# wells-wood-research/timed-design

Measured on AMD Instinct MI355X. Metric: residue_frames_per_sec, higher is better.
Workload: dtype f32

## Files before the change

### include/timed_hip.h

```cpp
#ifndef TIMED_HIP_H
#define TIMED_HIP_H

#include <stddef.h>
#include <stdint.h>

#ifdef __cplusplus
extern "C" {
#endif

#define TH_OK 0
#define TH_EINVAL (-1)
#define TH_EIO (-2)
#define TH_EHIP (-3)
#define TH_EUNSUP (-4)
#define TH_ENOMEM (-5)
#define TH_ECOMM (-6)
#define TH_EBUSY (-7)

#define TH_F32 0
#define TH_F64 1
#define TH_U8 2
#define TH_BOOL 3
#define TH_F16 4

#define TH_LOAD_DEFAULT 0u
#define TH_LOAD_NO_FUSE 1u
#define TH_LOAD_NO_MFMA 2u
#define TH_LOAD_KEEP_ALL 4u

#define TH_PREDICT_DEFAULT 0u
#define TH_PREDICT_LOGITS 1u
#define TH_PREDICT_OUT_DEVICE 2u
#define TH_PREDICT_IN_DEVICE 4u

typedef struct th_model th_model;
typedef struct th_comm th_comm;

int th_version(void);
const char* th_last_error(void);
int th_device_count(int* n_out);
int th_host_cpus(void);
int th_device_info(int device, char* name, size_t name_len, char* arch, size_t arch_len, int* cus);

int th_model_load(const char* pack_path, int device, unsigned flags, th_model** out);
int th_model_load_mem(const void* pack, size_t nbytes, int device, unsigned flags, th_model** out);
void th_model_free(th_model* m);
int th_model_info(const th_model* m, int dims[4], int* n_classes);
int th_model_cost(const th_model* m, double* algo_flops, double* exec_flops, int* n_steps);
int th_model_set_chunk(th_model* m, int frames_per_chunk);
int th_conv_gl_row_tiles(int64_t rows);

int th_predict(th_model* m, const void* frames, int dtype, int64_t n, float* probs_out, unsigned flags);
int th_predict_async(th_model* m, const void* frames, int dtype, int64_t n, float* probs_out, unsigned flags, int* ticket);
int th_predict_wait(th_model* m, int ticket);
#define TH_SPARSE_MAGIC "THSPF001"
int th_predict_sparse_async(th_model* m, const void* blob, size_t blob_bytes, float* probs_out, unsigned flags, int* ticket);
int th_host_alloc(size_t bytes, void** out);
int th_host_free(void* p);
int th_host_register(void* p, size_t bytes);
int th_host_unregister(void* p);
int th_predict_device(th_model* m, const void* d_frames, int dtype, int64_t n, float* d_probs, unsigned flags);
int th_model_fetch(th_model* m, const char* layer_name, int64_t n, float* out, int64_t out_floats);

int th_model_profile(th_model* m, int enable);
int th_model_step_info(const th_model* m, int i, char* label, size_t label_len, double* ms, int64_t* launches,
                       double* flops_per_frame, double* exec_flops_per_frame, double* bytes_per_frame);
int th_model_step_direct_flops(const th_model* m, int i, double* direct_flops_per_frame);

int th_model_guard_info(const th_model* m, int* state, double* max_dlogit, double* logit_scale, char* note, size_t note_len);

int th_model_knobs(const th_model* m, char* buf, size_t buf_len);

int th_dev_alloc(int device, size_t bytes, void** d_out);
int th_dev_free(int device, void* d);
int th_dev_upload(int device, void* d_dst, const void* h_src, size_t bytes);
int th_dev_download(int device, void* h_dst, const void* d_src, size_t bytes);
int th_dev_sync(int device);
int th_dev_synth_frames(int device, float* d_frames, int64_t n, int side, int channels, int atoms, uint64_t seed);

int th_apply_temp(const double* probs, int64_t n_res, int n_cls, double t, double* out);
int th_apply_temp_on(int device, const double* probs, int64_t n_res, int n_cls, double t, double* out);
#define TH_RNG_HOST 0
#define TH_RNG_PHILOX 1
// ... 134 lines not shown
```

### timed-design_amd/csrc/common.h

```cpp
#pragma once
#include <hip/hip_runtime.h>
#include <stdint.h>
#include <string>
#include <vector>

#include "../../include/timed_hip.h"

enum : int {
    OP_INPUT = 0, OP_CONV3D, OP_DENSE, OP_BN, OP_ACT, OP_MAXPOOL, OP_AVGPOOL, OP_GAP, OP_GMP,
    OP_FLATTEN, OP_CONCAT, OP_ADD, OP_IDENTITY
};
enum : int { ACT_LINEAR = 0, ACT_RELU, ACT_ELU, ACT_SOFTMAX, ACT_SIGMOID, ACT_TANH, ACT_LEAKY };

void th_set_error(const char* fmt, ...);
#define TH_FAIL(code, ...)          \
    do {                            \
        th_set_error(__VA_ARGS__);  \
        return (code);              \
    } while (0)
#define HIP_TRY(expr)                                                                            \
    do {                                                                                         \
        hipError_t _e = (expr);                                                                  \
        if (_e != hipSuccess) {                                                                  \
            th_set_error("%s failed: %s (%s:%d)", #expr, hipGetErrorString(_e), __FILE__, __LINE__); \
// ... 2 lines not shown
    } while (0)

#ifndef TH_KNOCKOUTS
#define TH_KNOCKOUTS 0
#endif
#if TH_KNOCKOUTS
#define TH_KNOCK_FIELD int dbg;
#define TH_KNOCK(a) ((a).dbg)
#define TH_KNOCK_SET(a, v) ((a).dbg = (v))
#else
#define TH_KNOCK_FIELD
#define TH_KNOCK(a) 0
#define TH_KNOCK_SET(a, v) ((void)0)
#endif

struct ThKnobs {
    int winograd = 1;
    int wino_split = 1;
    int wfused = 1;
    int wf_split = 1;
    int lanes = 1, lane_lag = 1;
    int guard = 1;
    int first_wino = 1;
    int first_split = 1;
    int conv_gl = 1;
    int dense_gemm = 1;
    int first_int = 1;
    int no_pool_first = 0;
    int no_tail_fuse = 0;
    int conv_notail = 0, n16_resident = 0;
    int wf_resident = 0, wf_noblk = 0;
    long long wino_piece = 0;
    int wino_b3var = 2, wino_nomid = 0;
#if TH_KNOCKOUTS
    int wf_dbg = 0, first_dbg = 0, wino_dbg = 0, conv_dbg = 0, pw_dbg = 0;
#endif
    std::string nondefault;
};
int th_knobs_read(ThKnobs* k);
inline const ThKnobs& th_knobs_of(const ThKnobs* k) { static const ThKnobs dflt; return k ? *k : dflt; }

hipError_t th_malloc_retry_impl(void** p, size_t bytes);
template <class T> inline hipError_t th_malloc_retry(T** p, size_t bytes) { return th_malloc_retry_impl(reinterpret_cast<void**>(p), bytes); }

int th_usable_cpus();

struct TView {
    float* p = nullptr;
    int D = 1, H = 1, W = 1, C = 0;
    int cs = 0;
    int coff = 0;
    int64_t fs = 0;
    int blk = 0;
    int V() const { return D * H * W; }
};

#define TH_MAX_POST 4
enum : int { POP_ACT = 1, POP_AFFINE = 2 };
struct PostOps {
    int n = 0;
    int type[TH_MAX_POST] = {0, 0, 0, 0};
    int act[TH_MAX_POST] = {0, 0, 0, 0};
    float alpha[TH_MAX_POST] = {0, 0, 0, 0};
    const float* scale[TH_MAX_POST] = {nullptr, nullptr, nullptr, nullptr};
    const float* shift[TH_MAX_POST] = {nullptr, nullptr, nullptr, nullptr};
    int monotone = 0;
// ... 62 lines not shown
int launch_conv_mfma(hipStream_t s, int64_t n, const ConvMfmaPlan& p, TView in, TView out, ConvGeom g, int Cin,
                     int Cout, const float* wpk, const float* bias, PreOp pre, PostOps post);

struct ConvN16Plan {
    int variant = -1, xc = 0;
    int pool = 0;
    int FB = 1, ZB = 0, nzb = 1;
    int Zp = 0, Hp = 0, Wp = 0;
    int Dc = 0, Hc = 0, Wc = 0;
    int rows_pf = 0, nchunks = 0;
    int geo = 0;
    int ncu = 0;
    size_t lds_bytes = 0, wpk_floats = 0;
    double exec_flops = 0;
    const ThKnobs* knobs = nullptr;
    std::string label;
};
bool conv_n16_plan(const TView& in, const TView& out_conv, const ConvGeom& g, int Cin, int Cout, int pool, const ThKnobs& kn, ConvN16Plan* plan);
void conv_n16_pack_weights(const ConvN16Plan& p, int Cin, int Cout, const float* w_keras, float* dst);
int launch_conv_n16(hipStream_t s, int64_t n, const ConvN16Plan& p, TView in, TView out, ConvGeom g, int Cin, int Cout, const float* wpk,
                    const float* bias, PreOp pre, PostOps post);

struct ConvWinoPlan {
    int P = 9;
    int Cin = 0, Cout = 0, Coutp = 0, ncb = 0;
    int Cinp = 0;
    size_t wpk_floats = 0;
    int64_t v_fpf = 0, m_fpf = 0;
    double gemm_flops = 0;
    double exec_flops = 0;
    int split = 0;
    int narrow = 0;
    int b3var = 0;
    const ThKnobs* knobs = nullptr;
    std::string label;
};
bool conv_wino_plan(const TView& in, const TView& out_conv, const ConvGeom& g, int Cin, int Cout, int scheme, int split, const ThKnobs& kn,
                    ConvWinoPlan* plan);
void conv_wino_pack_weights(const ConvWinoPlan& p, const float* w_keras, float* dst);
int launch_wino_in(hipStream_t s, int64_t n, const ConvWinoPlan& p, TView in, float* V, PreOp pre);
int launch_wino_gemm(hipStream_t s, int64_t n, const ConvWinoPlan& p, const float* V, float* M, const float* wpk);
int launch_wino_out(hipStream_t s, int64_t n, const ConvWinoPlan& p, const float* M, TView out, const float* bias, PostOps post, bool gap = false);
int launch_wino_mid(hipStream_t s, int64_t n, const ConvWinoPlan& p, const float* M, float* V_next, const float* bias, PostOps post);

struct ConvWfPlan {
    int geo = -1;
    int pool = 0;
    int Cin = 0, Cout = 0, ncb = 0, nchunks = 0;
    size_t wpk_floats = 0, lds_bytes = 0;
    double own_flops = 0;
    double exec_flops = 0;
    int ncu = 0;
    const ThKnobs* knobs = nullptr;
    std::string label;
};
bool conv_wf_plan(const TView& in, const TView& out_conv, const ConvGeom& g, int Cin, int Cout, int pool, const ThKnobs& kn, ConvWfPlan* plan);
bool conv_wf_view_ok(const TView& in);
int conv_wf_pre_kind(const PreOp& pre);
std::string conv_wf_label(const ConvWfPlan& p, const PreOp& pre);
void conv_wf_pack_weights(const ConvWfPlan& p, const float* w_keras, float* dst);
int launch_conv_wf(hipStream_t s, int64_t n, const ConvWfPlan& p, TView in, TView out, const float* wpk, const float* bias, PreOp pre,
                   PostOps post);

struct ConvWfsPlan {
    int geo = -1, pool = 0;
    int Cin = 0, Cout = 0, nkh = 0, ncp = 0;
    size_t wpk_floats = 0, lds_bytes = 0;
    double own_flops = 0, exec_flops = 0;
    int ncu = 0;
// ... 68 lines not shown
```

### timed-design_amd/csrc/conv_wino.hip

```cpp
#include "bf16x3.h"
#include "common.h"
#include "device_math.h"
#include "wino_tables.h"

#include <algorithm>
#include <cstdlib>
#include <cstring>
#include <thread>
#include <vector>

namespace {

constexpr int kZ = WINO_N;
constexpr int kNF = 64;
constexpr int kKC = 32;
constexpr int kCB = 128;

template <int R, int C>
__device__ __forceinline__ void wino_apply(const float (&T)[R][C], const float (&in)[C], float (&out)[R]) {
#pragma unroll
    for (int r = 0; r < R; ++r) {
        float acc = 0.f;
        bool first = true;
#pragma unroll
// ... 213 lines not shown
                th_act_vec<kZ * kZ>(y, a.post.act[i], a.post.alpha[i]);
            }
        }
        float u[kP][kZ];
#pragma unroll
        for (int k = 0; k < kZ; ++k) {
            float col[kZ], o[kP];
#pragma unroll
            for (int j = 0; j < kZ; ++j) col[j] = y[j * kZ + k];
            WinoTab<kP>::fwd(col, o);
#pragma unroll
            for (int aa = 0; aa < kP; ++aa) u[aa][k] = o[aa];
        }
        float* __restrict__ opos = a.V + (int64_t)z * kPos * opstride;
#pragma unroll
        for (int aa = 0; aa < kP; ++aa) {
            float o[kP];
            WinoTab<kP>::fwd(u[aa], o);
#pragma unroll
            for (int b = 0; b < kP; ++b) (opos + (int64_t)(aa * kP + b) * opstride)[ooff] = o[b];
        }
    }
}

struct WinoGemmArgs {
    const float* V; const float* U; float* M;
    int64_t Ns;
    int Cin, Coutp;
    int Cout;
    int nfb, ncb;
    int npos;
    unsigned total;
    unsigned per_xcd;
    TH_KNOCK_FIELD
};

__device__ __forceinline__ constexpr bool wino_tap_ok(int zi, int dz) { return zi - dz + 1 >= 0 && zi - dz + 1 < kZ; }

struct WinoTile {
    unsigned p, fb, cb;
    int lane, wave;
    bool active;
};

__device__ __forceinline__ bool wino_tile_index(const WinoGemmArgs& a, unsigned& L) {
    const unsigned xcd = blockIdx.x & 7u, slot = blockIdx.x >> 3;
    L = xcd * a.per_xcd + slot;
    return slot < a.per_xcd && L < a.total;
}
__device__ __forceinline__ WinoTile wino_tile(const WinoGemmArgs& a, unsigned L) {
    WinoTile t;
    t.cb = L % (unsigned)a.ncb;
    t.fb = (L / (unsigned)a.ncb) % (unsigned)a.nfb;
    t.p = L / (unsigned)(a.ncb * a.nfb);
    t.lane = threadIdx.x & 63;
    t.wave = __builtin_amdgcn_readfirstlane(threadIdx.x >> 6);
    t.active = (int)(t.cb * kCB) + t.wave * 32 < a.Cout;
    return t;
}

__global__ void __launch_bounds__(256, 2) k_wino_gemm(const WinoGemmArgs a) {
    __shared__ __attribute__((aligned(16))) float lds[kZ * kNF * kKC];
    unsigned L;
    if (!wino_tile_index(a, L)) return;
    const WinoTile t = wino_tile(a, L);
    const unsigned p = t.p, fb = t.fb, cb = t.cb;
    const int lane = t.lane, wave = t.wave;
    const int j = lane & 31, h = lane >> 5;
    const int nchunks = a.Cin / kKC;
    const int S = a.Cin / 8;
    const float4* wq = reinterpret_cast<const float4*>(a.U) + ((size_t)((p * a.ncb + cb) * 4 + wave) * S * 3) * 64 + lane;
    const float* vbase = a.V + ((int64_t)p * a.Ns + (int64_t)fb * kNF) * a.Cin;
    const int64_t zstride = (int64_t)a.npos * a.Ns * a.Cin;

    f32x16 acc[kZ][2];
#pragma unroll
    for (int z = 0; z < kZ; ++z)
#pragma unroll
        for (int rt = 0; rt < 2; ++rt)
#pragma unroll
            for (int r = 0; r < 16; ++r) acc[z][rt][r] = 0.f;
// ... 85 lines not shown
            for (int r = 0; r < 16; ++r) T[((r & 3) + 8 * (r >> 2) + 4 * h) * 36 + j] = acc[z][rt][r];
#pragma unroll
            for (int k = 0; k < 4; ++k) {
                const int row = rr + 8 * k;
                *reinterpret_cast<float4*>(mb + z * mz + (int64_t)(rt * 32 + row) * a.Coutp) = *reinterpret_cast<const float4*>(T + row * 36 + c4);
            }
        }
}


constexpr int kB3Slab = kZ * kNF * kKC * 2;
__device__ constexpr int kWinoPA[6] = {2, 0, 1, 1, 0, 0}, kWinoPB[6] = {0, 2, 1, 0, 1, 0};

__device__ __forceinline__ void wino_stage_split(const WinoGemmArgs& a, const __amdgpu_buffer_rsrc_t (&vrsrc)[kZ], unsigned goff, unsigned rstride32_b,
                                                 int ch, unsigned char* sdst) {
    float4 x[10];
#pragma unroll
    for (int i = 0; i < 10; ++i)
        x[i] = (TH_KNOCK(a) & 1) ? make_float4(1.f, 2.f, 3.f, 4.f) :
               __builtin_bit_cast(float4, __builtin_amdgcn_raw_buffer_load_b128(vrsrc[i >> 1], goff, (i & 1) * rstride32_b + ch * (kKC * 4), 0));
    __builtin_amdgcn_sched_barrier(0);
#pragma unroll
    for (int i = 0; i < 10; ++i) {
        uint2 h, m, l;
        bf16x3::split(x[i], h, m, l);
        *reinterpret_cast<uint2*>(sdst + i * 2048) = h;
        *reinterpret_cast<uint2*>(sdst + i * 2048 + kB3Slab) = m;
        *reinterpret_cast<uint2*>(sdst + i * 2048 + 2 * kB3Slab) = l;
    }
}

__device__ __forceinline__ constexpr int wino_b3_sw16(int R) { return ((R >> 2) & 3) ^ (((R >> 2) & 1) << 1); }

__global__ void __launch_bounds__(256, 2) k_wino_gemm_b3_16(const WinoGemmArgs a) {
    __shared__ __attribute__((aligned(16))) unsigned char lds[3 * kB3Slab];
    unsigned L;
    if (!wino_tile_index(a, L)) return;
    const WinoTile t = wino_tile(a, L);
    const int lane = t.lane;
    const int r16 = lane & 15, g16 = lane >> 4;
    const int nchunks = a.Cin / kKC;
    const __amdgpu_buffer_rsrc_t wrsrc = __builtin_amdgcn_make_buffer_rsrc(
        const_cast<float*>(a.U + ((size_t)((t.p * a.ncb + t.cb) * 4 + t.wave) * nchunks * 18) * 256), 0, 0xffffffffu, 0x00020000);
    const unsigned woff = (unsigned)lane * 16u;

    f32x4 acc[kZ][4][2];
#pragma unroll
    for (int z = 0; z < kZ; ++z)
#pragma unroll
        for (int rt = 0; rt < 4; ++rt)
#pragma unroll
            for (int ct = 0; ct < 2; ++ct) acc[z][rt][ct] = (f32x4){0.f, 0.f, 0.f, 0.f};

    const float* vbase = a.V + ((int64_t)t.p * a.Ns + (int64_t)t.fb * kNF) * a.Cin;
    const int64_t zstride = (int64_t)a.npos * a.Ns * a.Cin;
    __amdgpu_buffer_rsrc_t vrsrc[kZ];
#pragma unroll
    for (int z = 0; z < kZ; ++z) vrsrc[z] = __builtin_amdgcn_make_buffer_rsrc(const_cast<float*>(vbase + z * zstride), 0, 0xffffffffu, 0x00020000);
    const int r0 = 8 * t.wave + (lane >> 3), g4 = lane & 7;
    const unsigned goff = (unsigned)(r0 * a.Cin + 4 * g4) * 4u;
    const unsigned rstride32_b = (unsigned)(32 * a.Cin * 4);
    unsigned char* const sdst = lds + r0 * 64 + (((g4 >> 1) ^ wino_b3_sw16(r0)) << 4) + ((g4 & 1) << 3);
    const unsigned char* const aptr = lds + r16 * 64 + ((g16 ^ wino_b3_sw16(r16)) << 4);

    uint4 bw[2][3][3];
    auto load_b = [&](int ch, int ct) {
        if (TH_KNOCK(a) & 4) {
            const unsigned k = woff ^ ((unsigned)(ch * 2 + ct) << 4);
#pragma unroll
            for (int dz = 0; dz < 3; ++dz)
#pragma unroll
                for (int pc = 0; pc < 3; ++pc)
                    bw[ct][dz][pc] = make_uint4(0x3f813f82u ^ (k << (dz + pc)), 0x3e833e84u ^ k, 0x3d853d86u + (k << pc), 0x3c873c88u ^ (k << dz));
            return;
        }
#pragma unroll
        for (int dz = 0; dz < 3; ++dz)
#pragma unroll
            for (int pc = 0; pc < 3; ++pc)
                bw[ct][dz][pc] = __builtin_bit_cast(uint4, __builtin_amdgcn_raw_buffer_load_b128(wrsrc, woff, (((ch * 2 + ct) * 3 + dz) * 3 + pc) * 1024, 0));
    };

    for (int ch = 0; ch < nchunks; ++ch) {
        __syncthreads();
        wino_stage_split(a, vrsrc, goff, rstride32_b, ch, sdst);
        load_b(ch, 0);
        load_b(ch, 1);
        __syncthreads();
        if (!t.active) continue;
#pragma unroll
        for (int zi = 0; zi < kZ; ++zi)
#pragma unroll
            for (int rt = 0; rt < 4; ++rt) {
                bf16x8 af[3];
#pragma unroll
                for (int pc = 0; pc < 3; ++pc)
                    af[pc] = __builtin_bit_cast(bf16x8, *reinterpret_cast<const uint4*>(aptr + pc * kB3Slab + (zi * kNF + rt * 16) * 64));
#pragma unroll
                for (int dz = 0; dz < 3; ++dz) {
                    if (!wino_tap_ok(zi, dz)) continue;
                    const int zo = zi - dz + 1;
#pragma unroll
                    for (int c = 0; c < 6; ++c)
#pragma unroll
                        for (int ct = 0; ct < 2; ++ct)
                            acc[zo][rt][ct] = __builtin_amdgcn_mfma_f32_16x16x32_bf16(af[kWinoPA[c]], __builtin_bit_cast(bf16x8, bw[ct][dz][kWinoPB[c]]),
                                                                                     acc[zo][rt][ct], 0, 0, 0);
                }
                __builtin_amdgcn_sched_barrier(0);
            }
    }
    if (!t.active) return;
    if (TH_KNOCK(a) & 2) {
        float sum = 0.f;
#pragma unroll
        for (int z = 0; z < kZ; ++z)
#pragma unroll
            for (int rt = 0; rt < 4; ++rt)
#pragma unroll
                for (int ct = 0; ct < 2; ++ct)
#pragma unroll
                    for (int r = 0; r < 4; ++r) sum += acc[z][rt][ct][r];
        if (sum == 12345.678f) a.M[0] = sum;
        return;
    }
    __syncthreads();
    float* T = reinterpret_cast<float*>(lds) + t.wave * (16 * 36);
    const int rr = lane >> 3, c4 = (lane & 7) * 4;
    float* mb = a.M + ((int64_t)t.p * a.Ns + (int64_t)t.fb * kNF) * a.Coutp + t.cb * kCB + t.wave * 32 + c4;
    const int64_t mz = (int64_t)a.npos * a.Ns * a.Coutp;
#pragma unroll
    for (int z = 0; z < kZ; ++z)
#pragma unroll
        for (int rt = 0; rt < 4; ++rt) {
#pragma unroll
            for (int ct = 0; ct < 2; ++ct)
#pragma unroll
                for (int r = 0; r < 4; ++r) T[(4 * g16 + r) * 36 + ct * 16 + r16] = acc[z][rt][ct][r];
#pragma unroll
            for (int k = 0; k < 2; ++k) {
                const int row = rr + 8 * k;
                *reinterpret_cast<float4*>(mb + z * mz + (int64_t)(rt * 16 + row) * a.Coutp) = *reinterpret_cast<const float4*>(T + row * 36 + c4);
            }
        }
}

__global__ void __launch_bounds__(256, 2) k_wino_gemm_b3_32(const WinoGemmArgs a) {
    __shared__ __attribute__((aligned(16))) unsigned char lds[3 * kB3Slab];
    unsigned L;
    if (!wino_tile_index(a, L)) return;
    const WinoTile t = wino_tile(a, L);
    const int lane = t.lane;
    const int j = lane & 31, h = lane >> 5;
    const int nchunks = a.Cin / kKC;
    const int S = nchunks * 6;
    const uint4* wq = reinterpret_cast<const uint4*>(a.U) + ((size_t)((t.p * a.ncb + t.cb) * 4 + t.wave) * S * 3) * 64 + lane;

    f32x16 acc[kZ][2];
#pragma unroll
    for (int z = 0; z < kZ; ++z)
#pragma unroll
        for (int rt = 0; rt < 2; ++rt)
#pragma unroll
            for (int r = 0; r < 16; ++r) acc[z][rt][r] = 0.f;

    uint4 bw[2][3];
#pragma unroll
    for (int pc = 0; pc < 3; ++pc) bw[0][pc] = wq[pc * 64];
    const float* vbase = a.V + ((int64_t)t.p * a.Ns + (int64_t)t.fb * kNF) * a.Cin;
    const int64_t zstride = (int64_t)a.npos * a.Ns * a.Cin;
    __amdgpu_buffer_rsrc_t vrsrc[kZ];
#pragma unroll
    for (int z = 0; z < kZ; ++z) vrsrc[z] = __builtin_amdgcn_make_buffer_rsrc(const_cast<float*>(vbase + z * zstride), 0, 0xffffffffu, 0x00020000);
    const int r0 = 8 * t.wave + (lane >> 3), g4 = lane & 7;
    const unsigned goff = (unsigned)(r0 * a.Cin + 4 * g4) * 4u;
    const unsigned rstride32_b = (unsigned)(32 * a.Cin * 4);
    unsigned char* const sdst = lds + r0 * 64 + (((g4 >> 1) ^ ((r0 >> 2) & 3)) << 4) + ((g4 & 1) << 3);
// ... 287 lines not shown

static int64_t wino_piece(const ConvWinoPlan& p, int64_t n, int64_t Ns, int64_t fs, int width) {
    const int64_t lim = (1ll << 31) - 1;
    if (Ns * width > lim) return 0;
    const int64_t forced = th_knobs_of(p.knobs).wino_piece;
    const int64_t piece = std::max<int64_t>(1, std::min<int64_t>(n, lim / std::max<int64_t>(fs, 1)));
    return forced > 0 ? std::min(piece, forced) : piece;
}

int launch_wino_in(hipStream_t s, int64_t n, const ConvWinoPlan& p, TView in, float* V, PreOp pre) {
    if (n <= 0) return TH_OK;
    const int64_t Ns = (n + kNF - 1) / kNF * kNF;
    const int64_t piece = wino_piece(p, n, Ns, in.fs, p.Cinp);
    if (!piece) TH_FAIL(TH_EUNSUP, "conv_wino: %lld frames per launch exceed the 32-bit offsets of the transform kernels", (long long)n);
    const bool has_pre = pre.scale || pre.act != ACT_LINEAR;
    for (int64_t f0 = 0; f0 < n; f0 += piece) {
        const int64_t cnt = std::min(piece, n - f0);
        WinoInArgs ia;
        ia.in = in.p + f0 * in.fs; ia.in_fs = in.fs; ia.in_cs = in.cs; ia.in_coff = in.coff; ia.Cin = p.Cinp; ia.Creal = p.Cin; ia.pre = pre;
        ia.V = V + f0 * p.Cinp; ia.Ns = Ns; ia.n = cnt;
        const dim3 grid((unsigned)((cnt * p.Cinp + 255) / 256));
        if (p.P == 9) {
            if (has_pre) hipLaunchKernelGGL((k_wino_in<true, 9>), grid, dim3(256), 0, s, ia);
            else hipLaunchKernelGGL((k_wino_in<false, 9>), grid, dim3(256), 0, s, ia);
        } else {
            if (has_pre) hipLaunchKernelGGL((k_wino_in<true, 7>), grid, dim3(256), 0, s, ia);
            else hipLaunchKernelGGL((k_wino_in<false, 7>), grid, dim3(256), 0, s, ia);
        }
    }
    HIP_TRY(hipGetLastError());
    return TH_OK;
}

int launch_wino_gemm(hipStream_t s, int64_t n, const ConvWinoPlan& p, const float* V, float* M, const float* wpk) {
    if (n <= 0) return TH_OK;
    WinoGemmArgs ga;
    ga.V = V; ga.U = wpk; ga.M = M; ga.Ns = (n + kNF - 1) / kNF * kNF; ga.Cin = p.Cinp; ga.Coutp = p.Coutp;
    ga.Cout = p.Cout;
    ga.nfb = (int)(ga.Ns / kNF); ga.ncb = p.ncb;
    ga.npos = p.P * p.P;
    ga.total = (unsigned)(ga.npos * ga.nfb * ga.ncb);
    ga.per_xcd = (ga.total + 7) / 8;
    TH_KNOCK_SET(ga, th_knobs_of(p.knobs).wino_dbg);
    if (p.narrow) {
        const int64_t groups = (ga.Ns / 32 + 3) / 4;
        hipLaunchKernelGGL(k_wino_gemm_n32, dim3((unsigned)(ga.npos * groups)), dim3(256), 0, s, ga);
    } else if (p.split) {
        if (p.b3var == 2) hipLaunchKernelGGL(k_wino_gemm_b3_16, dim3(ga.per_xcd * 8), dim3(256), 0, s, ga);
        else hipLaunchKernelGGL(k_wino_gemm_b3_32, dim3(ga.per_xcd * 8), dim3(256), 0, s, ga);
    }
    else hipLaunchKernelGGL(k_wino_gemm, dim3(ga.per_xcd * 8), dim3(256), 0, s, ga);
    HIP_TRY(hipGetLastError());
    return TH_OK;
}

int launch_wino_out(hipStream_t s, int64_t n, const ConvWinoPlan& p, const float* M, TView out, const float* bias, PostOps post, bool gap) {
    if (n <= 0) return TH_OK;
    const int64_t Ns = (n + kNF - 1) / kNF * kNF;
    const int64_t piece = wino_piece(p, n, Ns, out.fs, p.Coutp);
    if (!piece) TH_FAIL(TH_EUNSUP, "conv_wino: %lld frames per launch exceed the 32-bit offsets of the transform kernels", (long long)n);
    for (int64_t f0 = 0; f0 < n; f0 += piece) {
        const int64_t cnt = std::min(piece, n - f0);
        WinoOutArgs oa;
        oa.M = M + f0 * p.Coutp; oa.Ns = Ns; oa.Coutp = p.Coutp; oa.Cout = p.Cout; oa.bias = bias; oa.post = post;
        oa.out = out.p + f0 * out.fs; oa.out_fs = out.fs; oa.out_cs = out.cs; oa.out_coff = out.coff; oa.n = cnt;
        const dim3 grid((unsigned)((cnt * p.Cout + 255) / 256));
        if (gap) {
            if (p.P == 9) hipLaunchKernelGGL((k_wino_out<9, true>), grid, dim3(256), 0, s, oa);
            else hipLaunchKernelGGL((k_wino_out<7, true>), grid, dim3(256), 0, s, oa);
        } else if (p.P == 9) hipLaunchKernelGGL(k_wino_out<9>, grid, dim3(256), 0, s, oa);
        else hipLaunchKernelGGL(k_wino_out<7>, grid, dim3(256), 0, s, oa);
    }
    HIP_TRY(hipGetLastError());
    return TH_OK;
}

int launch_wino_mid(hipStream_t s, int64_t n, const ConvWinoPlan& p, const float* M, float* V_next, const float* bias, PostOps post) {
    if (n <= 0) return TH_OK;
    const int64_t Ns = (n + kNF - 1) / kNF * kNF;
    if (Ns * (int64_t)p.Coutp >= (1ll << 31))
        TH_FAIL(TH_EUNSUP, "conv_wino: %lld frames per launch exceed the 32-bit offsets of the transform kernels", (long long)n);
// ... 12 lines not shown
```

### timed-design_amd/csrc/planner.hip

```cpp
#include "model.h"

#include <algorithm>
#include <cmath>
#include <cstring>
#include <map>
#include <set>

using namespace th_rt;

namespace {
struct PackNode {
    uint32_t op, n_in;
    int32_t in[kMaxIn];
    int32_t ip[kNIp];
    float fp[kNFp];
    int32_t w[kNW];
    char name[kNameBytes];
};
static_assert(sizeof(PackNode) == 256, "pack node record must be 256 bytes");
struct PackHeader {
    char magic[8];
    uint32_t n_nodes, n_blobs, output_node, reserved;
};

// ... 431 lines not shown
    }
    return TH_OK;
}

int choose_kernel(Planner& P, int i, LayerPlan& L) {
    th_model* m = P.m;
    if (int rc = build_epilogue(P, i, L)) return rc;
    const Node& n = P.N[i];
    const Node& sn = P.N[L.f.src];
    if (n.op == OP_DENSE) {
        if (sn.cs != sn.C || sn.coff != 0 || sn.D * sn.H * sn.W != 1) TH_FAIL(TH_EUNSUP, "%s: Dense needs a contiguous vector input", n.name.c_str());
        L.kind = P.kn.dense_gemm && dense_gemm_ok(sn.C, n.C, m->bufs[sn.buf].floats_per_frame) ? Kern::DenseGemm : Kern::Dense;
        return TH_OK;
    }
    const ConvGeom& g = L.g;
    const TView iv = shape_of(sn), ov = shape_of(n);
    const int Cin = sn.C, Cout = n.C;
    if (P.kn.winograd && P.use_mfma && P.fuse && L.f.pool < 0 && !L.split_softmax &&
        conv_wino_plan(iv, ov, g, Cin, Cout, P.kn.winograd == 2 ? 7 : 9, P.kn.wino_split, P.kn, &L.wp))
        L.kind = Kern::Wino;
    else if (L.wf && conv_wfs_plan(L.wfp, m->view(L.f.src), L.pre, P.kn, &L.sp)) L.kind = Kern::WfSplit;
    else if (L.wf) L.kind = Kern::Wf;
    else if (L.family == Kern::First5 || L.family == Kern::First || L.family == Kern::Pointwise) L.kind = L.family;
    else if (conv_gl_wanted(P.kn.conv_gl, g, n.D * n.H * n.W) && L.f.pool < 0 && !sn.blk && !P.N[L.f.last].blk &&
             L.family != Kern::N16 &&
             conv_gl_ok(Cin, Cout, sn.cs, sn.coff, (int64_t)m->bufs[sn.buf].floats_per_frame))
        L.kind = Kern::Gl;
    else if (L.family == Kern::N16) L.kind = Kern::N16;
    else if (L.family == Kern::Mfma) {
        L.kind = Kern::Mfma;
        L.tailed = conv_mfma_plan_tail(iv, ov, g, Cin, Cout, L.mp.pool, L.mp, P.kn, &L.tp, &L.cout_main);
    } else L.kind = Kern::Direct;
    if (L.kind == Kern::First) L.b3 = conv_first_b3_ok(L.fp, sn.D, sn.H, sn.W, Cin, std::min(Cout, 32), g, L.po);
    L.fp.ncu = L.np.ncu = L.wfp.ncu = L.sp.ncu = m->ncu;
    return TH_OK;
}

struct ConvArgs {
    th_model* M;
    int i, src, dst, Cin, Cout;
    ConvGeom g;
    const float* hw;
    const float* bias;
    PreOp pre;
    PostOps po;
    TView in() const { return M->view(src); }
    TView out() const { return M->view(dst); }
    const Node& node(int k) const { return M->nodes[k]; }
};

int emit_wino(Planner& P, const ConvArgs& c, const LayerPlan& L, Step st) {
    th_model* M = c.M;
    std::vector<Node>& N = P.N;
    const ConvWinoPlan wp = L.wp;
    float* dw;
    if (int rc = upload_packed(M, wp.wpk_floats, [&](float* d) { conv_wino_pack_weights(wp, c.hw, d); }, &dw)) return rc;
    if (M->wino_v_buf < 0) { M->wino_v_buf = P.new_buffer(0); M->wino_m_buf = P.new_buffer(0); }
    int64_t& v_fpf = M->bufs[M->wino_v_buf].floats_per_frame;
    v_fpf = std::max(v_fpf, wp.v_fpf);
    M->bufs[M->wino_m_buf].floats_per_frame = std::max(M->bufs[M->wino_m_buf].floats_per_frame, wp.m_fpf);
    const Node& sn = N[c.src];
    const double direct = st.flops, act_bytes = st.bytes, in_floats = (double)sn.D * sn.H * sn.W * c.Cin, mf = (double)wp.m_fpf;
    const std::string name = N[c.i].name, pts = std::to_string(wp.P * wp.P);
    auto Vp = [M]() { const Buffer& b = M->bufs[M->wino_v_buf]; return b.dev + M->lane.off * b.floats_per_frame; };
    auto Mp = [M]() { const Buffer& b = M->bufs[M->wino_m_buf]; return b.dev + M->lane.off * b.floats_per_frame; };
    if (!P.wino_in_done.count(c.i))
        P.add_step(st.out_node, name + ": wino_in (25 voxels -> " + pts + " points per plane) [k_wino_in]", 4.0 * (in_floats + (double)wp.v_fpf),
// ... 502 lines not shown
```

### timed-design_amd/csrc/runtime.hip

```cpp
#include "model.h"

#include <chrono>
#include <cstdarg>
#include <cstdio>
#include <cstring>

using namespace th_rt;

static thread_local char g_err[1024] = "";
void th_set_error(const char* fmt, ...) {
    va_list ap;
    va_start(ap, fmt);
    vsnprintf(g_err, sizeof g_err, fmt, ap);
    va_end(ap);
}

int th_knobs_read(ThKnobs* k) {
    *k = ThKnobs();
    std::string& nd = k->nondefault;
    auto note = [&](const char* name, const char* v) { nd += (nd.empty() ? "" : " "); nd += name; nd += "="; nd += v; };
    auto num = [&](const char* name, int* dst, int lo, int hi) {
        const char* e = getenv(name);
        if (!e) return;
        const int v = std::max(lo, std::min(hi, atoi(e)));
// ... 7 lines not shown
    const char* refused = nullptr;
#if TH_KNOCKOUTS
#define KNOCK(name, field) num(name, &k->field, 0, 1 << 20)
#else
    auto refuse = [&](const char* name) { const char* e = getenv(name); if (!refused && e && atoi(e) != 0) refused = name; };
#define KNOCK(name, field) refuse(name)
#endif
    num("TH_WINOGRAD", &k->winograd, 0, 2);
    num("TH_WINO_SPLIT", &k->wino_split, 0, 1);
    num("TH_WFUSED", &k->wfused, 0, 1);
    num("TH_WF_SPLIT", &k->wf_split, 0, 1);
    if (const char* e = getenv("TH_LANES")) { k->lanes = atoi(e) == 2 ? 2 : 1; if (k->lanes != 1) note("TH_LANES", e); }
    num("TH_LANE_LAG", &k->lane_lag, 0, 1 << 20);
    num("TH_GUARD", &k->guard, 0, 2);
    num("TH_FIRST_WINO", &k->first_wino, 0, 1);
    num("TH_FIRST_SPLIT", &k->first_split, 0, 1);
    num("TH_FIRST_INT", &k->first_int, 0, 1);
    num("TH_DENSE_GEMM", &k->dense_gemm, 0, 1);
    num("TH_CONV_GL", &k->conv_gl, 0, 2);
    KNOCK("TH_FIRST_DBG", first_dbg);
    flag("TH_NO_POOL_FIRST", &k->no_pool_first);
    flag("TH_NO_TAIL_FUSE", &k->no_tail_fuse);
    flag("TH_CONV_NOTAIL", &k->conv_notail);
    KNOCK("TH_CONV_DBG", conv_dbg);
    num("TH_N16_RESIDENT", &k->n16_resident, 0, 1 << 20);
    KNOCK("TH_PW_DBG", pw_dbg);
    num("TH_WF_RESIDENT", &k->wf_resident, 0, 1 << 20);
    KNOCK("TH_WF_DBG", wf_dbg);
    num("TH_WF_NOBLK", &k->wf_noblk, 0, 1);
    if (const char* e = getenv("TH_WINO_PIECE")) { k->wino_piece = std::max(0ll, atoll(e)); if (k->wino_piece) note("TH_WINO_PIECE", e); }
    KNOCK("TH_WINO_DBG", wino_dbg);
    num("TH_WINO_B3VAR", &k->wino_b3var, 0, 2);
    num("TH_WINO_NOMID", &k->wino_nomid, 0, 1);
#undef KNOCK
    if (refused)
        TH_FAIL(TH_EINVAL, "%s is set, but this library has no timing knock-outs: build the knock-out library "
                           "(tools/build_knockouts.py) and load it through TIMED_HIP_LIB", refused);
    return TH_OK;
}

int th_rt::load_common(th_model* m, const ThKnobs& knobs) {
    HIP_TRY(hipSetDevice(m->device));
    HIP_TRY(hipDeviceGetAttribute(&m->ncu, hipDeviceAttributeMultiprocessorCount, m->device));
    HIP_TRY(hipStreamCreateWithFlags(&m->stream, hipStreamNonBlocking));
    HIP_TRY(hipStreamCreateWithFlags(&m->pipe.copy_stream, hipStreamNonBlocking));
    HIP_TRY(hipStreamCreateWithFlags(&m->pipe.d2h_stream, hipStreamNonBlocking));
    HIP_TRY(hipStreamCreateWithFlags(&m->lane.stream2, hipStreamNonBlocking));
    HIP_TRY(hipEventCreateWithFlags(&m->lane.ev_fork, hipEventDisableTiming));
    HIP_TRY(hipEventCreateWithFlags(&m->lane.ev_join, hipEventDisableTiming));
    m->knobs = knobs;
    m->lane.lanes = m->knobs.lanes; m->lane.lag = m->knobs.lane_lag;
    for (int r = 0; r < th_model::kRing; ++r) {
        HIP_TRY(hipEventCreateWithFlags(&m->pipe.ev_h2d[r], hipEventDisableTiming));
        HIP_TRY(hipEventCreateWithFlags(&m->pipe.ev_free[r], hipEventDisableTiming));
    }
    for (th_model::Ticket& t : m->pipe.tickets) {
        HIP_TRY(hipEventCreateWithFlags(&t.computed, hipEventDisableTiming));
        HIP_TRY(hipEventCreateWithFlags(&t.done, hipEventDisableTiming));
    }
    int rc = parse_pack(m);
    if (rc) return rc;
    return plan(m);
}

th_model::~th_model() {
    (void)hipSetDevice(device);
// ... 231 lines not shown
```

### timed-design_amd/timed_hip/_lib.py

```python
from __future__ import annotations

import ctypes as C
import os

_HERE = os.path.dirname(os.path.abspath(__file__))
LIB_PATH = os.environ.get("TIMED_HIP_LIB", os.path.join(_HERE, "libtimedhip.so"))

TH_OK = 0
TH_EINVAL, TH_EIO, TH_EHIP, TH_EUNSUP, TH_ENOMEM, TH_ECOMM, TH_EBUSY = -1, -2, -3, -4, -5, -6, -7
TH_F32, TH_F64, TH_U8, TH_BOOL, TH_F16 = 0, 1, 2, 3, 4
TH_LOAD_DEFAULT, TH_LOAD_NO_FUSE, TH_LOAD_NO_MFMA, TH_LOAD_KEEP_ALL = 0, 1, 2, 4
TH_PREDICT_DEFAULT, TH_PREDICT_LOGITS, TH_PREDICT_OUT_DEVICE, TH_PREDICT_IN_DEVICE = 0, 1, 2, 4
TH_RNG_HOST, TH_RNG_PHILOX, TH_RNG_MT19937, TH_RNG_MT_WORDS = 0, 1, 2, 3
TH_TEMPER_NONE, TH_TEMPER_POW, TH_TEMPER_PREPOWERED = 0, 1, 2
TH_COMM_ID_BYTES = 128

_vp, _i, _u, _i64, _u64, _d, _sz = C.c_void_p, C.c_int, C.c_uint, C.c_int64, C.c_uint64, C.c_double, C.c_size_t
_pi, _pd, _pi64 = C.POINTER(C.c_int), C.POINTER(C.c_double), C.POINTER(C.c_int64)

PROTOTYPES = {
    "th_version": (_i, []),
    "th_last_error": (C.c_char_p, []),
    "th_device_count": (_i, [_pi]),
    "th_host_cpus": (_i, []),
    "th_device_info": (_i, [_i, C.c_char_p, _sz, C.c_char_p, _sz, _pi]),
    "th_model_load": (_i, [C.c_char_p, _i, _u, C.POINTER(_vp)]),
    "th_model_load_mem": (_i, [_vp, _sz, _i, _u, C.POINTER(_vp)]),
    "th_model_free": (None, [_vp]),
    "th_model_info": (_i, [_vp, C.POINTER(C.c_int * 4), _pi]),
    "th_model_cost": (_i, [_vp, _pd, _pd, _pi]),
    "th_model_set_chunk": (_i, [_vp, _i]),
    "th_conv_gl_row_tiles": (_i, [_i64]),
    "th_predict": (_i, [_vp, _vp, _i, _i64, _vp, _u]),
    "th_predict_device": (_i, [_vp, _vp, _i, _i64, _vp, _u]),
    "th_predict_async": (_i, [_vp, _vp, _i, _i64, _vp, _u, _pi]),
    "th_predict_sparse_async": (_i, [_vp, _vp, _sz, _vp, _u, _pi]),
    "th_predict_wait": (_i, [_vp, _i]),
    "th_host_alloc": (_i, [_sz, C.POINTER(_vp)]),
    "th_host_free": (_i, [_vp]),
    "th_host_register": (_i, [_vp, _sz]),
    "th_host_unregister": (_i, [_vp]),
    "th_model_fetch": (_i, [_vp, C.c_char_p, _i64, _vp, _i64]),
    "th_model_profile": (_i, [_vp, _i]),
    "th_model_step_info": (_i, [_vp, _i, C.c_char_p, _sz, _pd, _pi64, _pd, _pd, _pd]),
    "th_model_knobs": (_i, [_vp, C.c_char_p, _sz]),
    "th_model_step_direct_flops": (_i, [_vp, _i, _pd]),
    "th_model_guard_info": (_i, [_vp, C.POINTER(C.c_int), _pd, _pd, C.c_char_p, _sz]),
    "th_dev_alloc": (_i, [_i, _sz, C.POINTER(_vp)]),
    "th_dev_free": (_i, [_i, _vp]),
    "th_dev_upload": (_i, [_i, _vp, _vp, _sz]),
    "th_dev_download": (_i, [_i, _vp, _vp, _sz]),
    "th_dev_sync": (_i, [_i]),
    "th_dev_synth_frames": (_i, [_i, _vp, _i64, _i, _i, _i, _u64]),
    "th_apply_temp": (_i, [_vp, _i64, _i, _d, _vp]),
    "th_apply_temp_on": (_i, [_i, _vp, _i64, _i, _d, _vp]),
    "th_sampler_create": (_i, [_i, C.POINTER(_vp)]),
    "th_sampler_free": (None, [_vp]),
    "th_sampler_load": (_i, [_vp, _vp, _i64, _i, _d, _i, _i, _vp]),
    "th_sampler_draw": (_i, [_vp, _i64, _pi64, _i64, _i, _u64, _u64, _vp, C.c_char_p, _vp, _vp, _vp, _vp]),
    "th_sampler_uniform_buffer": (_i, [_vp, _sz, C.POINTER(C.c_void_p)]),
    "th_sampler_run": (_i, [_vp, _vp, _i64, _i, _i, _i64, _pi64, _i64, _i, _u64, _u64, _vp, C.c_char_p, C.c_uint, C.POINTER(C.c_void_p), _pi64]),
    "th_sample": (_i, [_vp, _i64, _i, _i64, _d, _i, _u64, _vp, _vp]),
    "th_sample_ex": (_i, [_vp, _i64, _i, _i64, _d, _i, _u64, _u64, _vp, _vp, _vp, C.c_char_p, _vp, _vp, _i]),
    "th_comm_unique_id": (_i, [C.c_char_p]),
    "th_comm_init": (_i, [C.c_char_p, _i, _i, _i, C.POINTER(_vp)]),
# ... 87 lines not shown
```

Measured before the change: 591,100.

## Split Winograd GEMM tail wave tiles into row parts to fill idle CUs

Computes how many b3_16 Winograd GEMM tiles fall into a partial last wave, given CU count and occupancy. When that remainder is under half the slots, those tiles are split into 2 or 4 row-part blocks, each handling 32 or 16 of the 64 frame rows. A templated body with fewer row tiles and a partial staging path serves these smaller blocks. The aim is to cut tail-wave load imbalance, at the cost of reloading weights per part and a more complex block-to-tile mapping.

```diff
diff --git a/include/timed_hip.h b/include/timed_hip.h
--- a/include/timed_hip.h
+++ b/include/timed_hip.h
@@ -49,6 +49,8 @@
 int th_model_cost(const th_model* m, double* algo_flops, double* exec_flops, int* n_steps);
 int th_model_set_chunk(th_model* m, int frames_per_chunk);
 int th_conv_gl_row_tiles(int64_t rows);
+int th_wino_tail_plan(int64_t total, int64_t slots, int qmask, int64_t* full_out, int* q_out);
+int th_wino_tail_block(int64_t total, int64_t slots, int qmask, int64_t block, int64_t* grid_out, int64_t* tile_out, int* part_out, int* q_out);
 
 int th_predict(th_model* m, const void* frames, int dtype, int64_t n, float* probs_out, unsigned flags);
 int th_predict_async(th_model* m, const void* frames, int dtype, int64_t n, float* probs_out, unsigned flags, int* ticket);
diff --git a/timed-design_amd/csrc/common.h b/timed-design_amd/csrc/common.h
--- a/timed-design_amd/csrc/common.h
+++ b/timed-design_amd/csrc/common.h
@@ -58,6 +58,8 @@
     int wf_resident = 0, wf_noblk = 0;
     long long wino_piece = 0;
     int wino_b3var = 2, wino_nomid = 0;
+    int wino_tail = 1;
+    int wino_slots = 0;
 #if TH_KNOCKOUTS
     int wf_dbg = 0, first_dbg = 0, wino_dbg = 0, conv_dbg = 0, pw_dbg = 0;
 #endif
@@ -186,9 +188,12 @@
     int split = 0;
     int narrow = 0;
     int b3var = 0;
-    const ThKnobs* knobs = nullptr;
-    std::string label;
-};
+    int ncu = 0;
+    const ThKnobs* knobs = nullptr;
+    std::string label;
+};
+struct WinoTail { int64_t full = 0; int q = 1; };
+WinoTail wino_tail_plan(int64_t total, int64_t slots, int qmask);
 bool conv_wino_plan(const TView& in, const TView& out_conv, const ConvGeom& g, int Cin, int Cout, int scheme, int split, const ThKnobs& kn,
                     ConvWinoPlan* plan);
 void conv_wino_pack_weights(const ConvWinoPlan& p, const float* w_keras, float* dst);
diff --git a/timed-design_amd/csrc/conv_wino.hip b/timed-design_amd/csrc/conv_wino.hip
--- a/timed-design_amd/csrc/conv_wino.hip
+++ b/timed-design_amd/csrc/conv_wino.hip
@@ -269,6 +269,8 @@
     int npos;
     unsigned total;
     unsigned per_xcd;
+    unsigned tail_wpx, tail_rq, tail_rr;
+    int tail_qs;
     TH_KNOCK_FIELD
 };
 
@@ -284,6 +286,27 @@
     const unsigned xcd = blockIdx.x & 7u, slot = blockIdx.x >> 3;
     L = xcd * a.per_xcd + slot;
     return slot < a.per_xcd && L < a.total;
+}
+__host__ __device__ __forceinline__ bool wino_tail_unit(unsigned block, unsigned total, unsigned per_xcd, unsigned wpx, unsigned rq, unsigned rr, int tail_qs,
+                                                        unsigned& L, unsigned& part, int& qs) {
+    const bool whole = block < wpx * 8u;
+    const unsigned b = whole ? block : block - wpx * 8u;
+    const unsigned xcd = b & 7u, slot = b >> 3;
+    const unsigned first = xcd * per_xcd;
+    const unsigned nx = first >= total ? 0u : (total - first < per_xcd ? total - first : per_xcd);
+    const unsigned want = rq + (xcd < rr ? 1u : 0u), rx = want < nx ? want : nx;
+    if (whole) {
+        part = 0; qs = 0;
+        L = first + slot;
+        return slot < nx - rx;
+    }
+    qs = tail_qs;
+    L = first + (nx - rx) + (slot >> qs);
+    part = slot & ((1u << qs) - 1u);
+    return slot < (rx << qs);
+}
+__device__ __forceinline__ bool wino_tile_part(const WinoGemmArgs& a, unsigned& L, unsigned& part, int& qs) {
+    return wino_tail_unit(blockIdx.x, a.total, a.per_xcd, a.tail_wpx, a.tail_rq, a.tail_rr, a.tail_qs, L, part, qs);
 }
 __device__ __forceinline__ WinoTile wino_tile(const WinoGemmArgs& a, unsigned L) {
     WinoTile t;
@@ -435,11 +458,29 @@
 
 __device__ __forceinline__ constexpr int wino_b3_sw16(int R) { return ((R >> 2) & 3) ^ (((R >> 2) & 1) << 1); }
 
-__global__ void __launch_bounds__(256, 2) k_wino_gemm_b3_16(const WinoGemmArgs a) {
-    __shared__ __attribute__((aligned(16))) unsigned char lds[3 * kB3Slab];
-    unsigned L;
-    if (!wino_tile_index(a, L)) return;
-    const WinoTile t = wino_tile(a, L);
+template <int RT>
+__device__ __forceinline__ void wino_stage_split_part(const WinoGemmArgs& a, const __amdgpu_buffer_rsrc_t (&vrsrc)[kZ], unsigned goff, int wave, int ch,
+                                                      unsigned char* sdst) {
+    if (wave >= 2 * RT) return;
+    float4 x[kZ];
+#pragma unroll
+    for (int z = 0; z < kZ; ++z)
+        x[z] = (TH_KNOCK(a) & 1) ? make_float4(1.f, 2.f, 3.f, 4.f) :
+               __builtin_bit_cast(float4, __builtin_amdgcn_raw_buffer_load_b128(vrsrc[z], goff, ch * (kKC * 4), 0));
+    __builtin_amdgcn_sched_barrier(0);
+#pragma unroll
+    for (int z = 0; z < kZ; ++z) {
+        uint2 h, m, l;
+        bf16x3::split(x[z], h, m, l);
+        *reinterpret_cast<uint2*>(sdst + z * 4096) = h;
+        *reinterpret_cast<uint2*>(sdst + z * 4096 + kB3Slab) = m;
+        *reinterpret_cast<uint2*>(sdst + z * 4096 + 2 * kB3Slab) = l;
+    }
+}
+
+template <int RT>
+__device__ __forceinline__ void wino_gemm_b3_16_body(const WinoGemmArgs& a, const WinoTile& t, unsigned part, unsigned char* lds) {
+    const unsigned prow = RT == 4 ? 0u : part * (16u * RT);
     const int lane = t.lane;
     const int r16 = lane & 15, g16 = lane >> 4;
     const int nchunks = a.Cin / kKC;
@@ -447,15 +488,15 @@
         const_cast<float*>(a.U + ((size_t)((t.p * a.ncb + t.cb) * 4 + t.wave) * nchunks * 18) * 256), 0, 0xffffffffu, 0x00020000);
     const unsigned woff = (unsigned)lane * 16u;
 
-    f32x4 acc[kZ][4][2];
+    f32x4 acc[kZ][RT][2];
 #pragma unroll
     for (int z = 0; z < kZ; ++z)
 #pragma unroll
-        for (int rt = 0; rt < 4; ++rt)
+        for (int rt = 0; rt < RT; ++rt)
 #pragma unroll
             for (int ct = 0; ct < 2; ++ct) acc[z][rt][ct] = (f32x4){0.f, 0.f, 0.f, 0.f};
 
-    const float* vbase = a.V + ((int64_t)t.p * a.Ns + (int64_t)t.fb * kNF) * a.Cin;
+    const float* vbase = a.V + ((int64_t)t.p * a.Ns + (int64_t)t.fb * kNF + prow) * a.Cin;
     const int64_t zstride = (int64_t)a.npos * a.Ns * a.Cin;
     __amdgpu_buffer_rsrc_t vrsrc[kZ];
 #pragma unroll
@@ -486,7 +527,8 @@
 
     for (int ch = 0; ch < nchunks; ++ch) {
         __syncthreads();
-        wino_stage_split(a, vrsrc, goff, rstride32_b, ch, sdst);
+        if constexpr (RT == 4) wino_stage_split(a, vrsrc, goff, rstride32_b, ch, sdst);
+        else wino_stage_split_part<RT>(a, vrsrc, goff, t.wave, ch, sdst);
         load_b(ch, 0);
         load_b(ch, 1);
         __syncthreads();
@@ -494,7 +536,7 @@
 #pragma unroll
         for (int zi = 0; zi < kZ; ++zi)
 #pragma unroll
-            for (int rt = 0; rt < 4; ++rt) {
+            for (int rt = 0; rt < RT; ++rt) {
                 bf16x8 af[3];
 #pragma unroll
                 for (int pc = 0; pc < 3; ++pc)
@@ -519,7 +561,7 @@
 #pragma unroll
         for (int z = 0; z < kZ; ++z)
 #pragma unroll
-            for (int rt = 0; rt < 4; ++rt)
+            for (int rt = 0; rt < RT; ++rt)
 #pragma unroll
                 for (int ct = 0; ct < 2; ++ct)
 #pragma unroll
@@ -530,12 +572,12 @@
     __syncthreads();
     float* T = reinterpret_cast<float*>(lds) + t.wave * (16 * 36);
     const int rr = lane >> 3, c4 = (lane & 7) * 4;
-    float* mb = a.M + ((int64_t)t.p * a.Ns + (int64_t)t.fb * kNF) * a.Coutp + t.cb * kCB + t.wave * 32 + c4;
+    float* mb = a.M + ((int64_t)t.p * a.Ns + (int64_t)t.fb * kNF + prow) * a.Coutp + t.cb * kCB + t.wave * 32 + c4;
     const int64_t mz = (int64_t)a.npos * a.Ns * a.Coutp;
 #pragma unroll
     for (int z = 0; z < kZ; ++z)
 #pragma unroll
-        for (int rt = 0; rt < 4; ++rt) {
+        for (int rt = 0; rt < RT; ++rt) {
 #pragma unroll
             for (int ct = 0; ct < 2; ++ct)
 #pragma unroll
@@ -546,6 +588,17 @@
                 *reinterpret_cast<float4*>(mb + z * mz + (int64_t)(rt * 16 + row) * a.Coutp) = *reinterpret_cast<const float4*>(T + row * 36 + c4);
             }
         }
+}
+
+__global__ void __launch_bounds__(256, 2) k_wino_gemm_b3_16(const WinoGemmArgs a) {
+    __shared__ __attribute__((aligned(16))) unsigned char lds[3 * kB3Slab];
+    unsigned L, part;
+    int qs;
+    if (!wino_tile_part(a, L, part, qs)) return;
+    const WinoTile t = wino_tile(a, L);
+    if (qs == 0) wino_gemm_b3_16_body<4>(a, t, 0u, lds);
+    else if (qs == 1) wino_gemm_b3_16_body<2>(a, t, part, lds);
+    else wino_gemm_b3_16_body<1>(a, t, part, lds);
 }
 
 __global__ void __launch_bounds__(256, 2) k_wino_gemm_b3_32(const WinoGemmArgs a) {
@@ -899,6 +952,57 @@
     return TH_OK;
 }
 
+WinoTail wino_tail_plan(int64_t total, int64_t slots, int qmask) {
+    WinoTail t;
+    const int64_t rem = total % slots;
+    t.full = total - rem;
+    if (rem == 0 || 2 * rem >= slots) return t;
+    for (int q = 4; q > 1; q >>= 1)
+        if ((qmask & q) && rem * q <= slots) { t.q = q; break; }
+    return t;
+}
+extern "C" int th_wino_tail_plan(int64_t total, int64_t slots, int qmask, int64_t* full_out, int* q_out) {
+    if (total < 0 || slots < 1 || !(qmask & 1) || !full_out || !q_out) TH_FAIL(TH_EINVAL, "th_wino_tail_plan: total >= 0, slots >= 1, a qmask with bit 1 and two outputs");
+    const WinoTail t = wino_tail_plan(total, slots, qmask);
+    *full_out = t.full; *q_out = t.q;
+    return TH_OK;
+}
+
+struct WinoTailGrid { unsigned per_xcd, wpx, rq, rr; int qs; unsigned blocks; };
+static WinoTailGrid wino_tail_grid(unsigned total, const WinoTail& t) {
+    WinoTailGrid g;
+    const unsigned rem = t.q > 1 ? total - (unsigned)t.full : 0u;
+    g.per_xcd = (total + 7) / 8;
+    g.rq = rem / 8; g.rr = rem % 8;
+    g.wpx = g.per_xcd - g.rq;
+    g.qs = t.q == 4 ? 2 : t.q == 2 ? 1 : 0;
+    g.blocks = (g.wpx + ((g.rq + (g.rr ? 1u : 0u)) << g.qs)) * 8;
+    return g;
+}
+extern "C" int th_wino_tail_block(int64_t total, int64_t slots, int qmask, int64_t block, int64_t* grid_out, int64_t* tile_out, int* part_out, int* q_out) {
+    if (total < 0 || total >= (1ll << 29) || slots < 1 || !(qmask & 1) || block < 0 || !grid_out || !tile_out || !part_out || !q_out)
+        TH_FAIL(TH_EINVAL, "th_wino_tail_block: 0 <= total < 2^29, slots >= 1, a qmask with bit 1, block >= 0 and four outputs");
+    const WinoTailGrid g = wino_tail_grid((unsigned)total, wino_tail_plan(total, slots, qmask));
+    *grid_out = g.blocks;
+    if (block >= g.blocks && !(block == 0 && g.blocks == 0)) TH_FAIL(TH_EINVAL, "th_wino_tail_block: block %lld of a grid of %u", (long long)block, g.blocks);
+    unsigned L = 0, part = 0;
+    int qs = 0;
+    const bool work = g.blocks && wino_tail_unit((unsigned)block, (unsigned)total, g.per_xcd, g.wpx, g.rq, g.rr, g.qs, L, part, qs);
+    *tile_out = work ? (int64_t)L : -1; *part_out = work ? (int)part : 0; *q_out = 1 << qs;
+    return work ? 1 : 0;
+}
+
+static int64_t wino_b3_16_slots(const ConvWinoPlan& p) {
+    const int64_t forced = th_knobs_of(p.knobs).wino_slots;
+    if (forced > 0) return forced;
+    static const int per_cu = [] {
+        int nb = 0;
+        if (hipOccupancyMaxActiveBlocksPerMultiprocessor(&nb, k_wino_gemm_b3_16, 256, 0) != hipSuccess) { (void)hipGetLastError(); nb = 2; }
+        return std::max(1, std::min(nb, 2));
+    }();
+    return (int64_t)std::max(1, p.ncu) * per_cu;
+}
+
 int launch_wino_gemm(hipStream_t s, int64_t n, const ConvWinoPlan& p, const float* V, float* M, const float* wpk) {
     if (n <= 0) return TH_OK;
     WinoGemmArgs ga;
@@ -908,12 +1012,19 @@
     ga.npos = p.P * p.P;
     ga.total = (unsigned)(ga.npos * ga.nfb * ga.ncb);
     ga.per_xcd = (ga.total + 7) / 8;
+    ga.tail_wpx = ga.per_xcd; ga.tail_rq = ga.tail_rr = 0; ga.tail_qs = 0;
     TH_KNOCK_SET(ga, th_knobs_of(p.knobs).wino_dbg);
     if (p.narrow) {
         const int64_t groups = (ga.Ns / 32 + 3) / 4;
         hipLaunchKernelGGL(k_wino_gemm_n32, dim3((unsigned)(ga.npos * groups)), dim3(256), 0, s, ga);
     } else if (p.split) {
-        if (p.b3var == 2) hipLaunchKernelGGL(k_wino_gemm_b3_16, dim3(ga.per_xcd * 8), dim3(256), 0, s, ga);
+        if (p.b3var == 2) {
+            if (th_knobs_of(p.knobs).wino_tail) {
+                const WinoTailGrid g = wino_tail_grid(ga.total, wino_tail_plan(ga.total, wino_b3_16_slots(p), 1 | 2 | 4));
+                ga.tail_wpx = g.wpx; ga.tail_rq = g.rq; ga.tail_rr = g.rr; ga.tail_qs = g.qs;
+            }
+            hipLaunchKernelGGL(k_wino_gemm_b3_16, dim3((ga.tail_wpx + ((ga.tail_rq + (ga.tail_rr ? 1u : 0u)) << ga.tail_qs)) * 8), dim3(256), 0, s, ga);
+        }
         else hipLaunchKernelGGL(k_wino_gemm_b3_32, dim3(ga.per_xcd * 8), dim3(256), 0, s, ga);
     }
     else hipLaunchKernelGGL(k_wino_gemm, dim3(ga.per_xcd * 8), dim3(256), 0, s, ga);
diff --git a/timed-design_amd/csrc/planner.hip b/timed-design_amd/csrc/planner.hip
--- a/timed-design_amd/csrc/planner.hip
+++ b/timed-design_amd/csrc/planner.hip
@@ -487,7 +487,7 @@
         L.tailed = conv_mfma_plan_tail(iv, ov, g, Cin, Cout, L.mp.pool, L.mp, P.kn, &L.tp, &L.cout_main);
     } else L.kind = Kern::Direct;
     if (L.kind == Kern::First) L.b3 = conv_first_b3_ok(L.fp, sn.D, sn.H, sn.W, Cin, std::min(Cout, 32), g, L.po);
-    L.fp.ncu = L.np.ncu = L.wfp.ncu = L.sp.ncu = m->ncu;
+    L.fp.ncu = L.np.ncu = L.wfp.ncu = L.sp.ncu = L.wp.ncu = m->ncu;
     return TH_OK;
 }
 
diff --git a/timed-design_amd/csrc/runtime.hip b/timed-design_amd/csrc/runtime.hip
--- a/timed-design_amd/csrc/runtime.hip
+++ b/timed-design_amd/csrc/runtime.hip
@@ -63,6 +63,8 @@
     KNOCK("TH_WINO_DBG", wino_dbg);
     num("TH_WINO_B3VAR", &k->wino_b3var, 0, 2);
     num("TH_WINO_NOMID", &k->wino_nomid, 0, 1);
+    num("TH_WINO_TAIL", &k->wino_tail, 0, 1);
+    num("TH_WINO_SLOTS", &k->wino_slots, 0, 1 << 20);
 #undef KNOCK
     if (refused)
         TH_FAIL(TH_EINVAL, "%s is set, but this library has no timing knock-outs: build the knock-out library "
diff --git a/timed-design_amd/timed_hip/_lib.py b/timed-design_amd/timed_hip/_lib.py
--- a/timed-design_amd/timed_hip/_lib.py
+++ b/timed-design_amd/timed_hip/_lib.py
@@ -31,6 +31,8 @@
     "th_model_cost": (_i, [_vp, _pd, _pd, _pi]),
     "th_model_set_chunk": (_i, [_vp, _i]),
     "th_conv_gl_row_tiles": (_i, [_i64]),
+    "th_wino_tail_plan": (_i, [_i64, _i64, _i, _pi64, _pi]),
+    "th_wino_tail_block": (_i, [_i64, _i64, _i, _i64, _pi64, _pi64, _pi, _pi]),
     "th_predict": (_i, [_vp, _vp, _i, _i64, _vp, _u]),
     "th_predict_device": (_i, [_vp, _vp, _i, _i64, _vp, _u]),
     "th_predict_async": (_i, [_vp, _vp, _i, _i64, _vp, _u, _pi]),
```

Result: no change. 595,100, median of 6 (+0.7%).
